# isl-org/Open3D-ML

Measured on AMD Instinct MI355X. Metric: point-cloud frames/sec (RandLA-Net SemanticKITTI inference: H2D + kNN pyramid + forward), higher is better.
Workload: dtype f32

## Files before the change

### include/ml3d_hip.h

```cpp
#ifndef ML3D_HIP_H
#define ML3D_HIP_H

#include <stddef.h>
#include <stdint.h>

#ifdef __cplusplus
extern "C" {
#endif

#define ML3D_OK 0
#define ML3D_E_INVALID (-1)
#define ML3D_E_WORKSPACE (-2)
#define ML3D_E_LAUNCH (-3)
#define ML3D_E_UNSUPPORTED (-4)

#define ML3D_ABI_VERSION 13
int ml3d_abi_version(void);

size_t ml3d_knn_workspace_bytes(int64_t n_points, int64_t n_queries, int64_t batch);

int ml3d_knn_search(const float* points, const int64_t* points_row_splits,
                    const float* queries, const int64_t* queries_row_splits,
                    int64_t batch, int64_t n_points, int64_t n_queries, int k,
                    int index_local, int32_t* out_index, float* out_dist2,
// ... 366 lines not shown
int ml3d_randla_knn_pyramid_ordered(const float* points, int64_t batch, int64_t n0, int num_layers,
                                    const int32_t* ratios_host, int k,
                                    int32_t* const* neighbor_idx_host, int32_t* const* interp_idx_host,
                                    int32_t* const* tile_order_host,
                                    void* workspace, size_t workspace_bytes, void* stream,
                                    const ml3d_trace* trace_host);

int ml3d_randla_forward_ordered(const ml3d_randla_desc* desc_host, const float* params,
                                const float* features, const float* points,
                                const int32_t* const* neighbor_idx_host,
                                const int32_t* const* interp_idx_host,
                                const int32_t* const* tile_order_host, float* out_scores,
                                void* workspace, size_t workspace_bytes, void* stream,
                                const ml3d_trace* trace_host);

int ml3d_gemm_tn(const float* a, int64_t lda, const float* b, int64_t ldb, int64_t m, int k, int n,
                 float* c, int64_t ldc, float* col_sums_a, void* stream);

size_t ml3d_batchnorm_train_workspace_bytes(int channels);

int ml3d_batchnorm_train_forward(const float* x, int64_t rows, int channels, const float* gamma,
                                 const float* beta, float eps, int act, float slope, float* y,
                                 float* save_mean, float* save_var, float* save_invstd,
                                 void* workspace, size_t workspace_bytes, void* stream);

int ml3d_batchnorm_train_backward(const float* x, const float* y, const float* grad_y, int64_t rows,
                                  int channels, const float* gamma, const float* save_mean,
                                  const float* save_invstd, int act, float slope, float* grad_x,
                                  float* grad_gamma, float* grad_beta, void* workspace,
                                  size_t workspace_bytes, void* stream);
// ... 118 lines not shown
```

### open3d-ml_amd/csrc/randla.hip

```cpp
#include <hip/hip_runtime.h>
#include <math.h>
#include <stdint.h>
#include <stdlib.h>

#include <type_traits>

#include "gemm.h"
#include <gfx950_ops.h>
#include "grid.h"
#include "ml3d_hip.h"

namespace ml3d {

static int64_t fuse_rows() {
#ifdef ML3D_TEST_HOOKS
    static const int64_t rows = [] { const char* e = getenv("ML3D_RANDLA_FUSE_ROWS"); return e ? (int64_t)atoll(e) : (int64_t)64 * 1024; }();
    return rows;
#else
    return 64 * 1024;
#endif
}

#ifndef ML3D_ATTN_B3
#define ML3D_ATTN_B3 3
// ... 24 lines not shown
struct LinArgs {
    const float* a0; int c0;
    const float* a1; int c1;
    const int32_t* gather;
    int64_t rows_per_item;
    int64_t a1_rows_per_item;
    const float* wt;
    const float* bias;
    const float* bias2;
    float* out;
    int64_t m_total;
    int cout;
    int act;
    float slope;
    void* pack_ws; size_t pack_bytes;
};

__global__ void __launch_bounds__(256)
head_fc0_mlp1(const float* __restrict__ x, int c0, const float* __restrict__ w0, const float* __restrict__ b0,
              const float* __restrict__ w1, const float* __restrict__ b1, int64_t m, float* __restrict__ feat,
              float* __restrict__ f1) {
    const int64_t i = (int64_t)blockIdx.x * blockDim.x + threadIdx.x;
    if (i >= m) return;
    float f[8], g[8];
#pragma unroll
    for (int c = 0; c < 8; ++c) f[c] = b0[c];
    const float* xr = x + i * c0;
    for (int j = 0; j < c0; ++j) {
        const float v = xr[j];
#pragma unroll
// ... 2226 lines not shown
    if (a.m_total <= 0) return 0;
    int64_t items = ((a.m_total + LIN_RM - 1) / LIN_RM) * a.cout;
    hipLaunchKernelGGL(linear_act, dim3((unsigned)((items + 255) / 256)), dim3(256), 0, st, a);
    return hipGetLastError() == hipSuccess ? 0 : ML3D_E_LAUNCH;
}

static int launch_linear_auto(const LinArgs& a, hipStream_t st) {
    if (!a.a1 && a.m_total >= fuse_rows()) {
        const ChainArgs c = chain_of(&a, 1);
        if (a.cout == 8 && mlp_shape_matches<ShapeLin16x8>(c)) return launch_mlp_wave_s<ShapeLin16x8, 8>(c, st);
        if (a.cout == 8 && mlp_shape_matches<ShapeLin8x8>(c)) return launch_mlp_wave_s<ShapeLin8x8, 8>(c, st);
        if (a.cout == 32 && mlp_shape_matches<ShapeLin64x32>(c)) return launch_mlp_wave_s<ShapeLin64x32, 8>(c, st);
        if (a.cout == 32 && mlp_shape_matches<ShapeLin32x32>(c)) return launch_mlp_wave_s<ShapeLin32x32, 8>(c, st);
        if (a.cout == 64 && mlp_shape_matches<ShapeLin32x64>(c)) return launch_mlp_wave_s<ShapeLin32x64, 8>(c, st);
    }
    if ((ML3D_LIN_B3_MINK) > 0 && a.pack_ws && !a.gather && a.c0 % 32 == 0 && (a.a1 ? a.c1 : 0) % 32 == 0 &&
        a.c0 + (a.a1 ? a.c1 : 0) >= (ML3D_LIN_B3_MINK) && a.cout % 4 == 0) {
        const int K = a.c0 + (a.a1 ? a.c1 : 0);
        const size_t need = gemm_pack_bf16x3_bytes(K, a.cout);
        if (need > 0 && need <= a.pack_bytes && gemm_pack_bf16x3(a.wt, K, a.cout, a.pack_ws, st) == 0) {
            const Epilogue ep = Epilogue::of(a.bias, a.act ? 1 : 0, a.slope).second_bias(a.bias2);
            const int rc = gemm_rows_bf16x3(a.a0, a.c0, a.c0, a.a1, a.c1, a.a1 ? a.c1 : 0, a.m_total, a.pack_ws, a.cout, ep, a.out,
                                            a.cout, nullptr, 0, st);
            if (rc != ML3D_E_UNSUPPORTED) return rc;
        }
    }
    if (a.c0 + a.c1 >= 8) {
        RowsA A;
        A.a = a.a0; A.lda = a.c0; A.k1 = a.c0;
        A.gather = a.a1 ? a.gather : nullptr; A.gather_stride = 1; A.a_rows = a.a1_rows_per_item;
        A.a2 = a.a1; A.lda2 = a.c1; A.k2 = a.a1 ? a.c1 : 0;
        A.gather_on_a2 = 1; A.g_rows_per_item = a.rows_per_item; A.g_src_rows_per_item = a.a1_rows_per_item;
        const Epilogue ep = Epilogue::of(a.bias, a.act ? 1 : 0, a.slope).second_bias(a.bias2);
        return gemm_rows(A, a.wt, a.m_total, a.cout, a.c0 + A.k2, ep, a.out, a.cout, nullptr, 0, st);
    }
    return launch_linear(a, st);
}
// ... 70 lines not shown
}

static size_t lin_pack_bytes(const ml3d_randla_desc* d) {
    size_t m = 0;
    int d_in = d->dim_features;
    for (int l = 0; l < d->num_layers; ++l) {
        const int dd = d->dim_output[l];
        const size_t a = gemm_pack_bf16x3_bytes(dd, dd), b = gemm_pack_bf16x3_bytes(dd + d_in, 2 * dd), c = gemm_pack_bf16x3_bytes(dd, dd / 2);
        m = a > m ? a : m; m = b > m ? b : m; m = c > m ? c : m;
        d_in = 2 * dd;
    }
    const size_t e = gemm_pack_bf16x3_bytes(d_in, d_in);
    return (e > m ? e : m) + 256;
}

static size_t fwd_ws_floats(const ml3d_randla_desc* d) {
    int64_t n[ML3D_RANDLA_MAX_LAYERS + 1];
    n[0] = d->num_points;
    for (int l = 0; l < d->num_layers; ++l) n[l + 1] = n[l] / d->sub_sampling_ratio[l];
    auto al = [](int64_t x) { return (x + 63) & ~(int64_t)63; };
    int64_t B = d->batch, f = 0;
    f += al(B * n[0] * d->dim_features);
    for (int l = 0; l < d->num_layers; ++l) {
        int64_t dd = d->dim_output[l], h = dd / 2;
        f += 2 * al(B * n[l] * h) + al(B * n[l] * 2 * dd) + al(B * n[l + 1] * 2 * dd) + 2 * al(B * n[l] * dd);
    }
    int64_t Dm = 2 * d->dim_output[d->num_layers - 1];
    f += al(B * n[d->num_layers] * Dm);
    int ed[ML3D_RANDLA_MAX_LAYERS + 1];
    enc_dims(d, ed);
    for (int i = 0; i < d->num_layers; ++i) {
        const int lev = d->num_layers - 1 - i, skip_c = ed[d->num_layers + 1 - i - 2];
        f += al(B * n[lev] * skip_c) + al(B * n[lev + 1] * skip_c);
    }
    f += al(B * n[0] * 64) + al(B * n[0] * 32);
    f += al((int64_t)(lin_pack_bytes(d) + 3) / 4) + 64;
    return (size_t)f;
}

}

using namespace ml3d;

extern "C" int ml3d_randla_param_layout(const ml3d_randla_desc* desc, int64_t* offsets_out, int max_slots) {
    if (!desc_ok(desc) || !offsets_out) return ML3D_E_INVALID;
    Layout L;
    make_layout(desc, &L);
    if (max_slots < L.n_slots + 1) return ML3D_E_INVALID;
    for (int i = 0; i <= L.n_slots; ++i) offsets_out[i] = L.off[i];
    return L.n_slots;
}

extern "C" size_t ml3d_randla_forward_workspace_bytes(const ml3d_randla_desc* desc) {
    if (!desc_ok(desc)) return 0;
    return fwd_ws_floats(desc) * 4 + 256;
}

extern "C" int ml3d_randla_forward(const ml3d_randla_desc* d, const float* params, const float* features,
                                   const float* points, const int32_t* const* neighbor_idx,
                                   const int32_t* const* interp_idx, float* out_scores, void* workspace,
                                   size_t workspace_bytes, void* stream) {
    return ml3d_randla_forward_traced(d, params, features, points, neighbor_idx, interp_idx, out_scores, workspace,
                                      workspace_bytes, stream, nullptr);
}

extern "C" int ml3d_randla_forward_traced(const ml3d_randla_desc* d, const float* params, const float* features,
                                          const float* points, const int32_t* const* neighbor_idx,
                                          const int32_t* const* interp_idx, float* out_scores, void* workspace,
                                          size_t workspace_bytes, void* stream, const ml3d_trace* trace) {
    return ml3d_randla_forward_ordered(d, params, features, points, neighbor_idx, interp_idx, nullptr, out_scores,
                                       workspace, workspace_bytes, stream, trace);
}

extern "C" int ml3d_randla_forward_ordered(const ml3d_randla_desc* d, const float* params, const float* features,
                                           const float* points, const int32_t* const* neighbor_idx,
                                           const int32_t* const* interp_idx, const int32_t* const* tile_order,
                                           float* out_scores, void* workspace, size_t workspace_bytes, void* stream,
                                           const ml3d_trace* trace) {
    if (!desc_ok(d) || !params || !features || !points || !neighbor_idx || !interp_idx || !out_scores)
        return ML3D_E_INVALID;
    if (d->num_neighbors != RK) return ML3D_E_UNSUPPORTED;
    if (workspace_bytes < ml3d_randla_forward_workspace_bytes(d)) return ML3D_E_WORKSPACE;
    hipStream_t st = (hipStream_t)stream;
    const Tracer T = {trace, st};
    const int Lr = d->num_layers;
    const int64_t B = d->batch;
    int64_t n[ML3D_RANDLA_MAX_LAYERS + 1];
    n[0] = d->num_points;
    for (int l = 0; l < Lr; ++l) n[l + 1] = n[l] / d->sub_sampling_ratio[l];
    if (n[Lr] < 1) return ML3D_E_INVALID;
    if (n[Lr - 1] < RK) return ML3D_E_UNSUPPORTED;
    Layout L;
    make_layout(d, &L);
    auto P = [&](int slot) { return params + L.off[slot]; };
    float* wsf = (float*)ws_align(workspace);
    auto take = [&](int64_t count) { float* p = wsf; wsf += (count + 63) & ~(int64_t)63; return p; };

    const size_t pack_bytes = lin_pack_bytes(d);
    void* pack_ws = take((int64_t)(pack_bytes + 3) / 4);
    auto lin = [&](const float* in, int k, int w, int b, float* out, int64_t rows, int cout, float slope,
                   const float* in1 = nullptr, int k1 = 0, int b2 = -1) {
        LinArgs a = {};
        a.pack_ws = pack_ws; a.pack_bytes = pack_bytes;
        a.a0 = in; a.c0 = k; a.a1 = in1; a.c1 = k1;
        a.wt = P(w); a.bias = b >= 0 ? P(b) : nullptr; a.bias2 = b2 >= 0 ? P(b2) : nullptr;
        a.out = out; a.m_total = rows; a.cout = cout; a.act = slope != 0.f; a.slope = slope;
        return a;
    };
    auto run = [&](int tag, const LinArgs& a) { return T.traced(tag, [&] { return launch_linear_auto(a, st); }); };
    int rc = 0;
    float* feat = take(B * n[0] * d->dim_features);
    float* f1_head = nullptr;
    if (d->dim_features == 8 && d->dim_output[0] == 16) {
        f1_head = take(B * n[0] * 8);
        const int64_t m = B * n[0];
        rc = T.traced(1000, [&] {
            hipLaunchKernelGGL(head_fc0_mlp1, dim3((unsigned)((m + 255) / 256)), dim3(256), 0, st, features, d->in_channels, P(0), P(1),
                               P(2), P(3), m, feat, f1_head);
// ... 100 lines not shown
    int cprev = Dm;
    for (int i = 0; i < Lr; ++i) {
        const int lev = Lr - 1 - i;
        const int skip_c = ed[Lr + 1 - i - 2];
        float* outp = take(B * n[lev] * skip_c);
        LinArgs a = lin(enc_keep[Lr + 1 - i - 2], skip_c, slot, slot + 1, outp, B * n[lev], skip_c, 0.2f, cur, cprev);
        a.gather = interp_idx[lev]; a.rows_per_item = n[lev]; a.a1_rows_per_item = n[lev + 1];
        if (i == Lr - 1) {
            LinArgs g[4] = {a};
            fc1(g + 1, outp, skip_c, nullptr, nullptr);
            const ChainArgs ch = chain_of(g, 4);
            if (mlp_shape_matches<ShapeDecFc1>(ch)) return T.traced(1200, [&] { return launch_chain_auto(ch, st); });
        }
        if (n[lev] >= 64 && (skip_c & 3) == 0 && (cprev & 3) == 0 && skip_c >= 8) {
            float* up = take(B * n[lev + 1] * skip_c);
            rc = T.traced(1100 + i, [&] {
                RowsA Au = {};
                Au.a = cur; Au.lda = cprev; Au.k1 = cprev;
                const int r = gemm_rows(Au, a.wt + (int64_t)skip_c * skip_c, B * n[lev + 1], skip_c, cprev, Epilogue{}, up, skip_c, nullptr, 0, st);
                if (r) return r;
                RowsA As = {};
                As.a = a.a0; As.lda = skip_c; As.k1 = skip_c;
                const Epilogue e1 = Epilogue::of(a.bias, 1, 0.2f).residual_rows(up, skip_c).gathered_residual(a.gather, 0, n[lev + 1], n[lev], n[lev + 1]);
                return gemm_rows(As, a.wt, a.m_total, skip_c, skip_c, e1, outp, skip_c, nullptr, 0, st);
            });
        } else {
            rc = run(1100 + i, a);
        }
        if (rc) return rc;
        slot += 2;
        cur = outp;
        cprev = skip_c;
    }
    float* t0 = take(B * n[0] * 64);
    float* t1 = take(B * n[0] * 32);
    LinArgs g[3];
    fc1(g, cur, cprev, t0, t1);
    return launch_linears(g, 3, true, T, 1200, st);
// ... 53 lines not shown
```

### open3d-ml_amd/ml3d/_abi.py

```python
import ctypes as C
import os

_HERE = os.path.dirname(os.path.abspath(__file__))
LIB_PATH = os.path.join(_HERE, "lib", "libml3d_hip.so")
MAX_LAYERS = 8
_lib = None

ERRORS = {-1: "invalid argument", -2: "workspace too small", -3: "HIP launch failed", -4: "unsupported configuration"}

ABI_VERSION = 13

SYMBOLS = [
    "ml3d_abi_version",
    "ml3d_knn_workspace_bytes",
    "ml3d_knn_search",
    "ml3d_radius_workspace_bytes",
    "ml3d_radius_count",
    "ml3d_radius_fill",
    "ml3d_radius_dense_workspace_bytes",
    "ml3d_radius_dense_gather",
    "ml3d_radius_dense_expand",
    "ml3d_ragged_to_dense",
    "ml3d_voxelize_workspace_bytes",
    "ml3d_voxelize_count",
# ... 44 lines not shown
    "ml3d_vote_update",
    "ml3d_randla_gather_max",
    "ml3d_randla_gather_max_backward",
    "ml3d_randla_attentive_pool",
    "ml3d_randla_attentive_pool_backward",
    "ml3d_argmax_labels",
    "ml3d_randla_pyramid_workspace_bytes",
    "ml3d_randla_knn_pyramid",
    "ml3d_randla_param_layout",
    "ml3d_randla_forward_workspace_bytes",
    "ml3d_randla_forward",
    "ml3d_randla_forward_traced",
    "ml3d_randla_knn_pyramid_traced",
    "ml3d_randla_knn_pyramid_ordered",
    "ml3d_randla_forward_ordered",
    "ml3d_gemm_tn",
    "ml3d_batchnorm_train_workspace_bytes", "ml3d_batchnorm_train_forward", "ml3d_batchnorm_train_backward",
    "ml3d_gather_rows", "ml3d_scatter_add_rows", "ml3d_gather_pool_backward",
    "ml3d_kpconv_deformed_weighted", "ml3d_kpconv_deformed_weighted_backward",
    "ml3d_kpconv_offset_regulariser_blocks", "ml3d_kpconv_offset_regulariser",
    "ml3d_randla_attention_stage", "ml3d_randla_attention_stage_backward_workspace_bytes", "ml3d_randla_attention_stage_backward",
    "ml3d_fps_workspace_bytes", "ml3d_furthest_point_sampling", "ml3d_pt_attention", "ml3d_pt_transition_down",
    "ml3d_pt_interpolate",
    "ml3d_pvcnn_voxel_coords", "ml3d_avg_voxelize_workspace_bytes", "ml3d_avg_voxelize", "ml3d_conv3d_ndhwc_bf16x3",
    "ml3d_trilinear_devoxelize", "ml3d_segment_max_rows_workspace_bytes", "ml3d_segment_max_rows",
    "ml3d_scn_build_workspace_bytes", "ml3d_scn_build", "ml3d_sparse_conv_bf16x3", "ml3d_scn_bn_relu",
    "ml3d_ball_query", "ml3d_pn2_sa_fused_supported", "ml3d_pn2_sa_mlp_max", "ml3d_pn2_group_rows", "ml3d_pn2_interpolate",
]


# ... 249 lines not shown
    lib.ml3d_randla_param_layout.restype = C.c_int
    lib.ml3d_randla_param_layout.argtypes = [C.POINTER(RandlaDesc), vp, i32]
    lib.ml3d_randla_forward_workspace_bytes.restype = sz
    lib.ml3d_randla_forward_workspace_bytes.argtypes = [C.POINTER(RandlaDesc)]
    lib.ml3d_randla_forward.restype = C.c_int
    lib.ml3d_randla_forward.argtypes = [C.POINTER(RandlaDesc), vp, vp, vp, vp, vp, vp, vp, sz, vp]
    lib.ml3d_randla_forward_traced.restype = C.c_int
    lib.ml3d_randla_forward_traced.argtypes = [C.POINTER(RandlaDesc), vp, vp, vp, vp, vp, vp, vp, sz, vp, C.POINTER(Trace)]
    lib.ml3d_randla_knn_pyramid_traced.restype = C.c_int
    lib.ml3d_randla_knn_pyramid_traced.argtypes = [vp, i64, i64, i32, vp, i32, vp, vp, vp, sz, vp, C.POINTER(Trace)]
    lib.ml3d_randla_knn_pyramid_ordered.restype = C.c_int
    lib.ml3d_randla_knn_pyramid_ordered.argtypes = [vp, i64, i64, i32, vp, i32, vp, vp, vp, vp, sz, vp, C.POINTER(Trace)]
    lib.ml3d_randla_forward_ordered.restype = C.c_int
    lib.ml3d_randla_forward_ordered.argtypes = [C.POINTER(RandlaDesc), vp, vp, vp, vp, vp, vp, vp, vp, sz, vp,
                                                C.POINTER(Trace)]
    return lib


def get():
    global _lib
    if _lib is None:
        if not os.path.exists(LIB_PATH):
            raise RuntimeError(
                "ml3d: %s is missing — build it with `python -c 'import __graft_entry__ as g; g.build()'` "
                "(hipcc --offload-arch=gfx950).  There is no CPU fallback." % LIB_PATH)
        lib = bind(C.CDLL(LIB_PATH))
        got = int(lib.ml3d_abi_version())
        if got != ABI_VERSION:
            raise RuntimeError("ml3d: %s has ABI version %d, this binding was written against %d (include/ml3d_hip.h) — rebuild "
                               "it with `python -c 'import __graft_entry__ as g; g.build()'`" % (LIB_PATH, got, ABI_VERSION))
# ... 69 lines not shown
```

### open3d-ml_amd/ml3d/engine.py

```python
import ctypes as C
import os

import torch

from . import _abi
from .ops import pyramid_sizes
from .torch.models import _randla_pack


class RandLAInferenceEngine:

    def __init__(self, cfg, state_dict, batch, num_points, device, tile_order=None):
        self.lib = _abi.get()
        if tile_order is None:
            env = (os.environ.get("ML3D_TILE_ORDER", "2") or "0").strip().lower()
            tile_order = True if env == "all" else int(env)
        self.tile_levels = (int(cfg["num_layers"]) if tile_order is True else int(tile_order or 0))
        self.tile_order = self.tile_levels > 0
        self.cfg = cfg
        self.device = torch.device(device)
        if self.device.type != "cuda":
            raise RuntimeError("RandLAInferenceEngine needs an MI355X device; there is no CPU fallback")
        self.B, self.N = int(batch), int(num_points)
        self.L = int(cfg["num_layers"])
        self.K = int(cfg["num_neighbors"])
        self.desc = _abi.make_desc(cfg, self.B, self.N)
        off = _abi.randla_param_offsets(self.lib, self.desc)
        self.params = torch.from_numpy(_randla_pack.pack(state_dict, cfg, off)).to(self.device)
        self.n = pyramid_sizes(self.N, cfg["sub_sampling_ratio"])
        dev = self.device
        self.nbr = [torch.empty((self.B, self.n[l], self.K), dtype=torch.int32, device=dev) for l in range(self.L)]
        self.itp = [torch.empty((self.B, self.n[l], 1), dtype=torch.int32, device=dev) for l in range(self.L)]
        self.scores = torch.empty((self.B, self.N, int(cfg["num_classes"])), dtype=torch.float32, device=dev)
        self.ratios = (C.c_int32 * self.L)(*[int(r) for r in cfg["sub_sampling_ratio"]])
        self.pyr_ws_bytes = self.lib.ml3d_randla_pyramid_workspace_bytes(self.B, self.N, self.L, self.ratios)
        self.fwd_ws_bytes = self.lib.ml3d_randla_forward_workspace_bytes(C.byref(self.desc))
        if self.pyr_ws_bytes == 0 or self.fwd_ws_bytes == 0:
            raise RuntimeError("RandLAInferenceEngine: invalid model/pyramid description")
        self.pyr_ws = torch.empty(self.pyr_ws_bytes, dtype=torch.uint8, device=dev)
        self.fwd_ws = torch.empty(self.fwd_ws_bytes, dtype=torch.uint8, device=dev)
        self._t_n = _abi.ptr_table([t.data_ptr() for t in self.nbr])
        self._t_i = _abi.ptr_table([t.data_ptr() for t in self.itp])
        self.order = [torch.empty(self.B * self.n[l], dtype=torch.int32, device=dev) if l < self.tile_levels else None
                      for l in range(self.L)] if self.tile_order else None
        self._t_o = _abi.ptr_table([0 if t is None else t.data_ptr() for t in self.order]) if self.tile_order else None

    def _check(self, points, features):
        if tuple(points.shape) != (self.B, self.N, 3) or points.dtype != torch.float32 or \
                not points.is_cuda or not points.is_contiguous():
            raise RuntimeError("engine: points must be a contiguous float32 CUDA tensor [%d, %d, 3]" % (self.B, self.N))
        if tuple(features.shape) != (self.B, self.N, int(self.cfg["in_channels"])) or \
                features.dtype != torch.float32 or not features.is_cuda or not features.is_contiguous():
            raise RuntimeError("engine: features must be a contiguous float32 CUDA tensor [B, N, in_channels]")

    def neighbors(self, points, trace=None):
        st = C.c_void_p(torch.cuda.current_stream().cuda_stream)
        rc = self.lib.ml3d_randla_knn_pyramid_ordered(points.data_ptr(), self.B, self.N, self.L, self.ratios, self.K,
                                                      self._t_n, self._t_i, self._t_o, self.pyr_ws.data_ptr(),
                                                      self.pyr_ws_bytes, st, trace)
        _abi.check(rc, "ml3d_randla_knn_pyramid")
        return self.nbr, self.itp

    def forward(self, points, features, trace=None):
        st = C.c_void_p(torch.cuda.current_stream().cuda_stream)
        rc = self.lib.ml3d_randla_forward_ordered(C.byref(self.desc), self.params.data_ptr(), features.data_ptr(),
                                                  points.data_ptr(), self._t_n, self._t_i, self._t_o,
                                                  self.scores.data_ptr(), self.fwd_ws.data_ptr(), self.fwd_ws_bytes, st,
                                                  trace)
        _abi.check(rc, "ml3d_randla_forward")
        return self.scores

    def step(self, points, features, knn_trace=None, fwd_trace=None):
        self._check(points, features)
        with torch.cuda.device(self.device):
            self.neighbors(points, knn_trace)
            return self.forward(points, features, fwd_trace)


class PipelinedRandLAEngine:

    def __init__(self, cfg, state_dict, batch, num_points, device):
        self.eng = [RandLAInferenceEngine(cfg, state_dict, batch, num_points, device) for _ in range(2)]
        self.eng[1].params = self.eng[0].params
        self.device = self.eng[0].device
        with torch.cuda.device(self.device):
            self.search = torch.cuda.Stream()
            self.compute = torch.cuda.Stream()
            self.knn_done = [torch.cuda.Event(), torch.cuda.Event()]
            self.fwd_done = [torch.cuda.Event(), torch.cuda.Event()]
            self.gate_tag = int(os.environ.get("ML3D_SEARCH_GATE", "9"))
            self.gate = [torch.cuda.Event(), torch.cuda.Event()]
            for g in self.gate:
                g.record()
        self.gate_rec = [None, None]
        self.i = 0
        self.n = self.eng[0].n

    def submit(self, points, features, knn_trace=None, fwd_trace=None, ready=None):
# ... 373 lines not shown
```

### open3d-ml_amd/ml3d/ops/__init__.py

```python
from ._gates import KnnResult, RadiusResult, VoxelizeResult
from .search import (knn_search, pyramid_sizes, randla_knn_pyramid, resolve_plans, fixed_radius_search,
                     radius_plan_dense, radius_fill_dense, radius_neighbors_dense, ragged_to_dense, _RadiusPlan,
                     _DenseRadiusPlan, kpconv_batch_build)
from .randla import randla_forward, GatherMaxFunction, AttentivePoolFunction
from .voxel import (voxelize, subsample_batch, subsample, rotate_points, grid_subsampling_plan,
                    batch_grid_subsampling, _SubsamplePlan)
from .kpconv import (kpconv_rigid, kpconv_deformable, linear, gather_pool, kpconv_weighted, kpconv_weighted_backward,
                     KPConvFunction)
from .detection import (pillar_features, conv2d_nhwc, pack_bf16x3, linear_bf16x3, deconv2d_nhwc, nhwc_to_nchw, nms, pointpillars_boxes,
                        iou_bev, iou_3d, topk_rows)
from .sampler import (nearest_to_center, argmax_labels, vote_update, device_patch, possibility_argmin,
                      device_patch_batch, sphere_select, device_sphere_batch)
from .train import (gemm_tn, LinearFunction, BatchNormActFunction, batch_norm_act, GatherRowsFunction, GatherPoolFunction,
                    AttentionStageFunction, attention_stage_supported, KPConvDeformedFunction, OffsetRegulariserFunction)
from .pointtransformer import furthest_point_sampling, pt_attention, pt_transition_down, pt_interpolate
from .pvcnn import (pvcnn_voxel_coords, avg_voxelize, pack_conv3d_weights, conv3d_ndhwc, trilinear_devoxelize,
                    segment_max_rows, linear_rows_bf16x3)
from .sparseconv import ScnPyramid, scn_build, pack_sparse_weights, sparse_conv, scn_bn_relu
from .pointnet2 import (ball_query, three_nn, three_interpolate, pn2_interpolate, pn2_sa_mlp_max, pack_sa_weights,
                        sa_fused)
```

### open3d-ml_amd/ml3d/ops/randla.py

```python
import ctypes as C

import numpy as np
import torch

from .. import _abi
from . import _gates
from ._gates import KnnResult, RadiusResult, VoxelizeResult, _splits, _splits_of_lengths


def _stream():
    return _gates._stream()


def _need_gpu(*tensors):
    return _gates._need_gpu(*tensors)


def _ws(nbytes, device):
    return _gates._ws(nbytes, device)

from .search import pyramid_sizes


def randla_forward(desc, params, features, points, neighbor_idx, interp_idx, out=None, workspace=None, tile_order=None):
    lib = _abi.get()
    _need_gpu(params, features, points, *neighbor_idx, *interp_idx)
    dev = points.device
    B, n0 = int(desc.batch), int(desc.num_points)
    if tuple(points.shape) != (B, n0, 3) or tuple(features.shape) != (B, n0, desc.in_channels):
        raise RuntimeError("randla_forward: points/features shape does not match the descriptor")
    for t in (points, features):
        if t.dtype != torch.float32 or not t.is_contiguous():
            raise RuntimeError("randla_forward: points/features must be contiguous float32")
    for t in list(neighbor_idx) + list(interp_idx):
        if t.dtype != torch.int32 or not t.is_contiguous():
            raise RuntimeError("randla_forward: index tensors must be contiguous int32")
    L, K = int(desc.num_layers), int(desc.num_neighbors)
    sizes = pyramid_sizes(n0, [int(desc.sub_sampling_ratio[i]) for i in range(L)])
    if len(neighbor_idx) != L or len(interp_idx) != L:
        raise RuntimeError("randla_forward: need %d neighbour and %d interpolation index tensors (got %d / %d)"
                           % (L, L, len(neighbor_idx), len(interp_idx)))
    for l in range(L):
        if tuple(neighbor_idx[l].shape) != (B, sizes[l], K):
            raise RuntimeError("randla_forward: neighbor_idx[%d] must be [%d, %d, %d], got %s"
                               % (l, B, sizes[l], K, tuple(neighbor_idx[l].shape)))
        if tuple(interp_idx[l].shape) not in ((B, sizes[l], 1), (B, sizes[l])):
            raise RuntimeError("randla_forward: interp_idx[%d] must be [%d, %d, 1], got %s"
                               % (l, B, sizes[l], tuple(interp_idx[l].shape)))
        if tile_order is not None and (l >= len(tile_order) or
                                       (tile_order[l] is not None and tile_order[l].numel() != B * sizes[l])):
            raise RuntimeError("randla_forward: tile_order[%d] must hold %d rows (or be None)" % (l, B * sizes[l]))
    if out is None:
        out = torch.empty((B, n0, desc.num_classes), dtype=torch.float32, device=dev)
    wsb = lib.ml3d_randla_forward_workspace_bytes(C.byref(desc))
    ws = workspace if workspace is not None else _ws(wsb, dev)
    if ws.numel() < wsb:
        raise RuntimeError("randla_forward: workspace too small")
    t_n = _abi.ptr_table([t.data_ptr() for t in neighbor_idx])
    t_i = _abi.ptr_table([t.data_ptr() for t in interp_idx])
    with torch.cuda.device(dev):
        if tile_order is not None:
            for t in tile_order:
                if t is not None and (t.dtype != torch.int32 or not t.is_contiguous() or t.device != dev):
                    raise RuntimeError("randla_forward: tile_order tensors must be contiguous int32 on the same device")
            t_o = _abi.ptr_table([0 if t is None else t.data_ptr() for t in tile_order])
            rc = lib.ml3d_randla_forward_ordered(C.byref(desc), params.data_ptr(), features.data_ptr(), points.data_ptr(),
                                                 t_n, t_i, t_o, out.data_ptr(), ws.data_ptr(), ws.numel(), _stream(), None)
        else:
            rc = lib.ml3d_randla_forward(C.byref(desc), params.data_ptr(), features.data_ptr(), points.data_ptr(),
                                         t_n, t_i, out.data_ptr(), ws.data_ptr(), ws.numel(), _stream())
    _abi.check(rc, "ml3d_randla_forward")
    return out


class GatherMaxFunction(torch.autograd.Function):

    @staticmethod
    def forward(ctx, features, neighbor_idx, n_out):
        lib = _abi.get()
        _need_gpu(features, neighbor_idx)
# ... 59 lines not shown
```

### open3d-ml_amd/ml3d/torch/models/randlanet.py

```python
import os

import numpy as np
import torch
import torch.nn as nn

from ... import _abi
from ... import ops
from . import _randla_pack
from ._datapath import GpuSearchTree, preprocess_segmentation
from ._multicloud import CloudSlots, PinnedUpload, check_many_args


class SharedMLP(nn.Module):

    def __init__(self, in_channels, out_channels, transpose=False, bn=True, activation_fn=None):
        super().__init__()
        conv = nn.ConvTranspose2d if transpose else nn.Conv2d
        self.conv = conv(in_channels, out_channels, kernel_size=1)
        self.batch_norm = nn.BatchNorm2d(out_channels, eps=1e-6, momentum=0.01) if bn else None
        self.activation_fn = activation_fn


class LocalSpatialEncoding(nn.Module):
    def __init__(self, dim_in, dim_out):
# ... 66 lines not shown
                                 SharedMLP(32, cfg.num_classes, bn=False))
        self._packed = None
        self._engines = {}
        self.use_graphs = os.environ.get("ML3D_RANDLA_GRAPHS", "0") == "1"
        self.eval()

    def _apply(self, fn, *a, **k):
        self._packed = None
        return super()._apply(fn, *a, **k)

    def load_state_dict(self, *a, **k):
        self._packed = None
        return super().load_state_dict(*a, **k)

    def packed_params(self, device):
        if self._packed is None or self._packed[0] != device:
            desc = _abi.make_desc(self.cfg, 1, max(self.cfg.num_points, 1))
            off = _abi.randla_param_offsets(_abi.get(), desc)
            buf = _randla_pack.pack(self.state_dict(), self.cfg, off)
            self._packed = (device, torch.from_numpy(buf).to(device))
        return self._packed[1]

    def invalidate_packed(self):
        self._packed = None

    def neighbor_pyramid(self, points):
        return ops.randla_knn_pyramid(points, self.cfg.sub_sampling_ratio, self.cfg.num_neighbors)

    def forward(self, inputs):
        if self.training:
            return self._forward_train(inputs)
        dev = self.device
        _abi.require_gpu(dev, "RandLANet.forward")
        fast = self._forward_graphed(inputs)
        if fast is not None:
# ... 3 lines not shown
        feat = inputs['features'].to(dev, torch.float32).contiguous()
        if 'neighbor_indices' in inputs and 'interp_idx' in inputs:
            nbr = [t.to(dev).to(torch.int32).contiguous() for t in inputs['neighbor_indices']]
            itp = [t.to(dev).to(torch.int32).contiguous() for t in inputs['interp_idx']]
            if 'sub_idx' in inputs:
                for l, (sub, nb) in enumerate(zip(inputs['sub_idx'], nbr)):
                    if getattr(sub, '_ml3d_prefix_of_neighbors', False) and sub.shape[-2] <= nb.shape[-2]:
                        continue
                    sub = sub.to(dev)
                    if sub.shape[-2] > nb.shape[-2] or not torch.equal(sub.to(torch.int32), nb[..., :sub.shape[-2], :]):
                        raise RuntimeError("RandLANet.forward: sub_idx[%d] is not the prefix of neighbor_indices[%d]" % (l, l))
        else:
            nbr, itp = self.neighbor_pyramid(pts)
        B, N, _ = pts.shape
        desc = _abi.make_desc(self.cfg, B, N)
        return ops.randla_forward(desc, self.packed_params(dev), feat, pts, nbr, itp)

    def _forward_graphed(self, inputs):
        st = getattr(self, '_dev_loop', None)
        feats = inputs.get('features') if isinstance(inputs, dict) else None
        mark = getattr(feats, '_ml3d_arena', None)
        if st is None or mark is None or not getattr(self, 'use_graphs', True) or st.get('fwd_failed') or st.get('layout') is None:
            return None
        arena, lay_id = mark
        lay, nbytes = st['layout']
        if lay_id != id(lay) or arena.numel() != nbytes or feats.dim() != 3 or feats.shape[0] != 1:
            return None
        base, L = arena.data_ptr(), int(self.cfg.num_layers)
        coords = inputs['coords'][0] if isinstance(inputs['coords'], (list, tuple)) else inputs['coords']
        try:
            ok = feats.data_ptr() == base + lay['feats'][0] and coords.data_ptr() == base + lay['pts'][0] and \
                all(inputs['neighbor_indices'][l].data_ptr() == base + lay['nbr%d' % l][0] and
                    inputs['interp_idx'][l].data_ptr() == base + lay['itp%d' % l][0] for l in range(L))
        except Exception:
            ok = False
        if not ok:
            return None
        dev = self.device
        fg = st.get('fwd_graph')
        params = self.packed_params(dev)
        if fg is not None and fg['params'] is not params:
            fg = None
        if fg is None:
            try:
                with torch.cuda.device(dev):
                    a_in = torch.empty(nbytes, dtype=torch.uint8, device=dev)
                    a_in.copy_(arena)
                    v = self._arena_views(a_in, lay)
                    k = int(self.cfg.num_points)
                    desc = _abi.make_desc(self.cfg, 1, k)
                    nbr = [v['nbr%d' % l] for l in range(L)]
                    itp = [v['itp%d' % l] for l in range(L)]
                    scores = torch.empty((1, k, int(self.cfg.num_classes)), dtype=torch.float32, device=dev)
                    run = lambda: ops.randla_forward(desc, params, v['feats'][None], v['pts'][None], nbr, itp, out=scores)
                    side = torch.cuda.Stream()
# ... 491 lines not shown
```

Baseline: 7560.

## Pre-pack RandLA-Net weights into bf16x3 planes once at load time

```diff
diff --git a/include/ml3d_hip.h b/include/ml3d_hip.h
--- a/include/ml3d_hip.h
+++ b/include/ml3d_hip.h
@@ -404,6 +404,19 @@
                                 void* workspace, size_t workspace_bytes, void* stream,
                                 const ml3d_trace* trace_host);
 
+size_t ml3d_randla_prepared_bytes(const ml3d_randla_desc* desc_host);
+int ml3d_randla_prepare(const ml3d_randla_desc* desc_host, const float* params, void* prepared, size_t prepared_bytes,
+                        void* stream);
+size_t ml3d_randla_prepared_forward_bytes(const ml3d_randla_desc* desc_host);
+int ml3d_randla_forward_prepared(const ml3d_randla_desc* desc_host, const float* params,
+                                 const float* features, const float* points,
+                                 const int32_t* const* neighbor_idx_host,
+                                 const int32_t* const* interp_idx_host,
+                                 const int32_t* const* tile_order_host, float* out_scores,
+                                 void* workspace, size_t workspace_bytes, void* stream,
+                                 const ml3d_trace* trace_host, const void* prepared, size_t prepared_bytes,
+                                 int32_t lin_min_k, int32_t dec_min_k);
+
 int ml3d_gemm_tn(const float* a, int64_t lda, const float* b, int64_t ldb, int64_t m, int k, int n,
                  float* c, int64_t ldc, float* col_sums_a, void* stream);
 
diff --git a/open3d-ml_amd/csrc/randla.hip b/open3d-ml_amd/csrc/randla.hip
--- a/open3d-ml_amd/csrc/randla.hip
+++ b/open3d-ml_amd/csrc/randla.hip
@@ -62,6 +62,7 @@
     int act;
     float slope;
     void* pack_ws; size_t pack_bytes;
+    const void* planes; int b3_min_k;
 };
 
 __global__ void __launch_bounds__(256)
@@ -2318,13 +2319,18 @@
         if (a.cout == 32 && mlp_shape_matches<ShapeLin32x32>(c)) return launch_mlp_wave_s<ShapeLin32x32, 8>(c, st);
         if (a.cout == 64 && mlp_shape_matches<ShapeLin32x64>(c)) return launch_mlp_wave_s<ShapeLin32x64, 8>(c, st);
     }
-    if ((ML3D_LIN_B3_MINK) > 0 && a.pack_ws && !a.gather && a.c0 % 32 == 0 && (a.a1 ? a.c1 : 0) % 32 == 0 &&
-        a.c0 + (a.a1 ? a.c1 : 0) >= (ML3D_LIN_B3_MINK) && a.cout % 4 == 0) {
+    if (!a.gather && a.c0 % 32 == 0 && (a.a1 ? a.c1 : 0) % 32 == 0 && a.cout % 4 == 0) {
         const int K = a.c0 + (a.a1 ? a.c1 : 0);
-        const size_t need = gemm_pack_bf16x3_bytes(K, a.cout);
-        if (need > 0 && need <= a.pack_bytes && gemm_pack_bf16x3(a.wt, K, a.cout, a.pack_ws, st) == 0) {
+        const void* planes = nullptr;
+        if (a.planes) {
+            if (K >= a.b3_min_k) planes = a.planes;
+        } else if ((ML3D_LIN_B3_MINK) > 0 && a.pack_ws && K >= (ML3D_LIN_B3_MINK)) {
+            const size_t need = gemm_pack_bf16x3_bytes(K, a.cout);
+            if (need > 0 && need <= a.pack_bytes && gemm_pack_bf16x3(a.wt, K, a.cout, a.pack_ws, st) == 0) planes = a.pack_ws;
+        }
+        if (planes) {
             const Epilogue ep = Epilogue::of(a.bias, a.act ? 1 : 0, a.slope).second_bias(a.bias2);
-            const int rc = gemm_rows_bf16x3(a.a0, a.c0, a.c0, a.a1, a.c1, a.a1 ? a.c1 : 0, a.m_total, a.pack_ws, a.cout, ep, a.out,
+            const int rc = gemm_rows_bf16x3(a.a0, a.c0, a.c0, a.a1, a.c1, a.a1 ? a.c1 : 0, a.m_total, planes, a.cout, ep, a.out,
                                             a.cout, nullptr, 0, st);
             if (rc != ML3D_E_UNSUPPORTED) return rc;
         }
@@ -2425,7 +2431,7 @@
     return (e > m ? e : m) + 256;
 }
 
-static size_t fwd_ws_floats(const ml3d_randla_desc* d) {
+static size_t fwd_ws_floats(const ml3d_randla_desc* d, bool pack) {
     int64_t n[ML3D_RANDLA_MAX_LAYERS + 1];
     n[0] = d->num_points;
     for (int l = 0; l < d->num_layers; ++l) n[l + 1] = n[l] / d->sub_sampling_ratio[l];
@@ -2445,13 +2451,87 @@
         f += al(B * n[lev] * skip_c) + al(B * n[lev + 1] * skip_c);
     }
     f += al(B * n[0] * 64) + al(B * n[0] * 32);
-    f += al((int64_t)(lin_pack_bytes(d) + 3) / 4) + 64;
-    return (size_t)f;
+    if (pack) f += al((int64_t)(lin_pack_bytes(d) + 3) / 4);
+    return (size_t)f + 64;
+}
+
+constexpr int PREP_LIN_MINK = 256;
+constexpr int PREP_DEC_MINK = INT32_MAX;
+constexpr int PREP_MINK = 64;
+
+struct PrepEntry { int slot, row0, K, N; void* planes; };
+struct RandlaPrepared {
+    int n;
+    PrepEntry e[6 * ML3D_RANDLA_MAX_LAYERS + 1 + 2 * ML3D_RANDLA_MAX_LAYERS];
+    const void* find(int slot, int row0, int K, int N) const {
+        for (int i = 0; i < n; ++i)
+            if (e[i].slot == slot && e[i].row0 == row0 && e[i].K == K && e[i].N == N) return e[i].planes;
+        return nullptr;
+    }
+};
+
+static RandlaPrepared randla_prepared_layout(WsLayout& L, const ml3d_randla_desc* d) {
+    RandlaPrepared P;
+    P.n = 0;
+    auto add = [&](int slot, int row0, int K, int N) {
+        if (K < PREP_MINK || (N & 3) != 0 || gemm_pack_bf16x3_bytes(K, N) == 0) return;
+        P.e[P.n++] = {slot, row0, K, N, L.take<char>(gemm_pack_bf16x3_bytes(K, N))};
+    };
+    int d_in = d->dim_features;
+    for (int l = 0; l < d->num_layers; ++l) {
+        const int dd = d->dim_output[l], h = dd / 2, sb = 2 + 18 * l;
+        add(sb + 0, 0, d_in, h);
+        add(sb + 4, 0, h, dd);
+        add(sb + 6, 0, dd, h);
+        add(sb + 10, 0, h, dd);
+        add(sb + 12, 0, dd, dd);
+        add(sb + 14, 0, dd + d_in, 2 * dd);
+        d_in = 2 * dd;
+    }
+    int slot = 2 + 18 * d->num_layers;
+    add(slot, 0, d_in, d_in);
+    slot += 2;
+    int ed[ML3D_RANDLA_MAX_LAYERS + 1];
+    enc_dims(d, ed);
+    int cprev = d_in;
+    for (int i = 0; i < d->num_layers; ++i) {
+        const int skip_c = ed[d->num_layers + 1 - i - 2];
+        add(slot, 0, skip_c, skip_c);
+        add(slot, skip_c, cprev, skip_c);
+        slot += 2;
+        cprev = skip_c;
+    }
+    return P;
 }
 
 }
 
 using namespace ml3d;
+
+extern "C" size_t ml3d_randla_prepared_bytes(const ml3d_randla_desc* desc) {
+    if (!desc_ok(desc)) return 0;
+    return ws_bytes_of(randla_prepared_layout, desc);
+}
+
+extern "C" int ml3d_randla_prepare(const ml3d_randla_desc* d, const float* params, void* prepared, size_t prepared_bytes,
+                                   void* stream) {
+    if (!desc_ok(d) || !params || !prepared) return ML3D_E_INVALID;
+    RandlaPrepared P;
+    if (!ws_carve(prepared, prepared_bytes, &P, randla_prepared_layout, d)) return ML3D_E_WORKSPACE;
+    Layout L;
+    make_layout(d, &L);
+    for (int i = 0; i < P.n; ++i) {
+        const PrepEntry& e = P.e[i];
+        const int rc = gemm_pack_bf16x3(params + L.off[e.slot] + (int64_t)e.row0 * e.N, e.K, e.N, e.planes, (hipStream_t)stream);
+        if (rc) return rc;
+    }
+    return 0;
+}
+
+extern "C" size_t ml3d_randla_prepared_forward_bytes(const ml3d_randla_desc* desc) {
+    if (!desc_ok(desc)) return 0;
+    return fwd_ws_floats(desc, false) * 4 + 256;
+}
 
 extern "C" int ml3d_randla_param_layout(const ml3d_randla_desc* desc, int64_t* offsets_out, int max_slots) {
     if (!desc_ok(desc) || !offsets_out) return ML3D_E_INVALID;
@@ -2464,7 +2544,7 @@
 
 extern "C" size_t ml3d_randla_forward_workspace_bytes(const ml3d_randla_desc* desc) {
     if (!desc_ok(desc)) return 0;
-    return fwd_ws_floats(desc) * 4 + 256;
+    return fwd_ws_floats(desc, true) * 4 + 256;
 }
 
 extern "C" int ml3d_randla_forward(const ml3d_randla_desc* d, const float* params, const float* features,
@@ -2483,15 +2563,41 @@
                                        workspace, workspace_bytes, stream, trace);
 }
 
+static int randla_forward(const ml3d_randla_desc* d, const float* params, const float* features, const float* points,
+                          const int32_t* const* neighbor_idx, const int32_t* const* interp_idx, const int32_t* const* tile_order,
+                          float* out_scores, void* workspace, size_t workspace_bytes, void* stream, const ml3d_trace* trace,
+                          const RandlaPrepared* prep, int lin_min_k, int dec_min_k);
+
 extern "C" int ml3d_randla_forward_ordered(const ml3d_randla_desc* d, const float* params, const float* features,
                                            const float* points, const int32_t* const* neighbor_idx,
                                            const int32_t* const* interp_idx, const int32_t* const* tile_order,
                                            float* out_scores, void* workspace, size_t workspace_bytes, void* stream,
                                            const ml3d_trace* trace) {
+    return randla_forward(d, params, features, points, neighbor_idx, interp_idx, tile_order, out_scores, workspace, workspace_bytes,
+                          stream, trace, nullptr, 0, 0);
+}
+
+extern "C" int ml3d_randla_forward_prepared(const ml3d_randla_desc* d, const float* params, const float* features,
+                                            const float* points, const int32_t* const* neighbor_idx,
+                                            const int32_t* const* interp_idx, const int32_t* const* tile_order,
+                                            float* out_scores, void* workspace, size_t workspace_bytes, void* stream,
+                                            const ml3d_trace* trace, const void* prepared, size_t prepared_bytes,
+                                            int32_t lin_min_k, int32_t dec_min_k) {
+    if (!desc_ok(d) || !prepared || lin_min_k < 0 || dec_min_k < 0) return ML3D_E_INVALID;
+    RandlaPrepared P;
+    if (!ws_carve((void*)prepared, prepared_bytes, &P, randla_prepared_layout, d)) return ML3D_E_WORKSPACE;
+    return randla_forward(d, params, features, points, neighbor_idx, interp_idx, tile_order, out_scores, workspace, workspace_bytes,
+                          stream, trace, &P, lin_min_k ? lin_min_k : PREP_LIN_MINK, dec_min_k ? dec_min_k : PREP_DEC_MINK);
+}
+
+static int randla_forward(const ml3d_randla_desc* d, const float* params, const float* features, const float* points,
+                          const int32_t* const* neighbor_idx, const int32_t* const* interp_idx, const int32_t* const* tile_order,
+                          float* out_scores, void* workspace, size_t workspace_bytes, void* stream, const ml3d_trace* trace,
+                          const RandlaPrepared* prep, int lin_min_k, int dec_min_k) {
     if (!desc_ok(d) || !params || !features || !points || !neighbor_idx || !interp_idx || !out_scores)
         return ML3D_E_INVALID;
     if (d->num_neighbors != RK) return ML3D_E_UNSUPPORTED;
-    if (workspace_bytes < ml3d_randla_forward_workspace_bytes(d)) return ML3D_E_WORKSPACE;
+    if (workspace_bytes < fwd_ws_floats(d, !prep) * 4 + 256) return ML3D_E_WORKSPACE;
     hipStream_t st = (hipStream_t)stream;
     const Tracer T = {trace, st};
     const int Lr = d->num_layers;
@@ -2507,12 +2613,13 @@
     float* wsf = (float*)ws_align(workspace);
     auto take = [&](int64_t count) { float* p = wsf; wsf += (count + 63) & ~(int64_t)63; return p; };
 
-    const size_t pack_bytes = lin_pack_bytes(d);
-    void* pack_ws = take((int64_t)(pack_bytes + 3) / 4);
+    const size_t pack_bytes = prep ? 0 : lin_pack_bytes(d);
+    void* pack_ws = prep ? nullptr : take((int64_t)(pack_bytes + 3) / 4);
     auto lin = [&](const float* in, int k, int w, int b, float* out, int64_t rows, int cout, float slope,
                    const float* in1 = nullptr, int k1 = 0, int b2 = -1) {
         LinArgs a = {};
         a.pack_ws = pack_ws; a.pack_bytes = pack_bytes;
+        if (prep) { a.planes = prep->find(w, 0, k + k1, cout); a.b3_min_k = lin_min_k; }
         a.a0 = in; a.c0 = k; a.a1 = in1; a.c1 = k1;
         a.wt = P(w); a.bias = b >= 0 ? P(b) : nullptr; a.bias2 = b2 >= 0 ? P(b2) : nullptr;
         a.out = out; a.m_total = rows; a.cout = cout; a.act = slope != 0.f; a.slope = slope;
@@ -2643,14 +2750,25 @@
         }
         if (n[lev] >= 64 && (skip_c & 3) == 0 && (cprev & 3) == 0 && skip_c >= 8) {
             float* up = take(B * n[lev + 1] * skip_c);
+            const void* up_planes = prep && cprev >= dec_min_k ? prep->find(slot, skip_c, cprev, skip_c) : nullptr;
+            const void* skip_planes = prep && skip_c >= dec_min_k ? prep->find(slot, 0, skip_c, skip_c) : nullptr;
             rc = T.traced(1100 + i, [&] {
-                RowsA Au = {};
-                Au.a = cur; Au.lda = cprev; Au.k1 = cprev;
-                const int r = gemm_rows(Au, a.wt + (int64_t)skip_c * skip_c, B * n[lev + 1], skip_c, cprev, Epilogue{}, up, skip_c, nullptr, 0, st);
+                int r = up_planes ? gemm_rows_bf16x3(cur, cprev, cprev, nullptr, 0, 0, B * n[lev + 1], up_planes, skip_c, Epilogue{}, up,
+                                                     skip_c, nullptr, 0, st)
+                                  : ML3D_E_UNSUPPORTED;
+                if (r == ML3D_E_UNSUPPORTED) {
+                    RowsA Au = {};
+                    Au.a = cur; Au.lda = cprev; Au.k1 = cprev;
+                    r = gemm_rows(Au, a.wt + (int64_t)skip_c * skip_c, B * n[lev + 1], skip_c, cprev, Epilogue{}, up, skip_c, nullptr, 0, st);
+                }
                 if (r) return r;
+                const Epilogue e1 = Epilogue::of(a.bias, 1, 0.2f).residual_rows(up, skip_c).gathered_residual(a.gather, 0, n[lev + 1], n[lev], n[lev + 1]);
+                r = skip_planes ? gemm_rows_bf16x3(a.a0, skip_c, skip_c, nullptr, 0, 0, a.m_total, skip_planes, skip_c, e1, outp, skip_c,
+                                                   nullptr, 0, st)
+                                : ML3D_E_UNSUPPORTED;
+                if (r != ML3D_E_UNSUPPORTED) return r;
                 RowsA As = {};
                 As.a = a.a0; As.lda = skip_c; As.k1 = skip_c;
-                const Epilogue e1 = Epilogue::of(a.bias, 1, 0.2f).residual_rows(up, skip_c).gathered_residual(a.gather, 0, n[lev + 1], n[lev], n[lev + 1]);
                 return gemm_rows(As, a.wt, a.m_total, skip_c, skip_c, e1, outp, skip_c, nullptr, 0, st);
             });
         } else {
diff --git a/open3d-ml_amd/ml3d/_abi.py b/open3d-ml_amd/ml3d/_abi.py
--- a/open3d-ml_amd/ml3d/_abi.py
+++ b/open3d-ml_amd/ml3d/_abi.py
@@ -82,6 +82,7 @@
     "ml3d_randla_knn_pyramid_traced",
     "ml3d_randla_knn_pyramid_ordered",
     "ml3d_randla_forward_ordered",
+    "ml3d_randla_prepared_bytes", "ml3d_randla_prepare", "ml3d_randla_prepared_forward_bytes", "ml3d_randla_forward_prepared",
     "ml3d_gemm_tn",
     "ml3d_batchnorm_train_workspace_bytes", "ml3d_batchnorm_train_forward", "ml3d_batchnorm_train_backward",
     "ml3d_gather_rows", "ml3d_scatter_add_rows", "ml3d_gather_pool_backward",
@@ -361,6 +362,15 @@
     lib.ml3d_randla_forward_ordered.restype = C.c_int
     lib.ml3d_randla_forward_ordered.argtypes = [C.POINTER(RandlaDesc), vp, vp, vp, vp, vp, vp, vp, vp, sz, vp,
                                                 C.POINTER(Trace)]
+    lib.ml3d_randla_prepared_bytes.restype = sz
+    lib.ml3d_randla_prepared_bytes.argtypes = [C.POINTER(RandlaDesc)]
+    lib.ml3d_randla_prepare.restype = C.c_int
+    lib.ml3d_randla_prepare.argtypes = [C.POINTER(RandlaDesc), vp, vp, sz, vp]
+    lib.ml3d_randla_prepared_forward_bytes.restype = sz
+    lib.ml3d_randla_prepared_forward_bytes.argtypes = [C.POINTER(RandlaDesc)]
+    lib.ml3d_randla_forward_prepared.restype = C.c_int
+    lib.ml3d_randla_forward_prepared.argtypes = [C.POINTER(RandlaDesc), vp, vp, vp, vp, vp, vp, vp, vp, sz, vp,
+                                                 C.POINTER(Trace), vp, sz, i32, i32]
     return lib
 
 
diff --git a/open3d-ml_amd/ml3d/engine.py b/open3d-ml_amd/ml3d/engine.py
--- a/open3d-ml_amd/ml3d/engine.py
+++ b/open3d-ml_amd/ml3d/engine.py
@@ -5,12 +5,13 @@
 
 from . import _abi
 from .ops import pyramid_sizes
+from .ops.randla import RandlaWeights, prepared_routing
 from .torch.models import _randla_pack
 
 
 class RandLAInferenceEngine:
 
-    def __init__(self, cfg, state_dict, batch, num_points, device, tile_order=None):
+    def __init__(self, cfg, state_dict, batch, num_points, device, tile_order=None, weights=None):
         self.lib = _abi.get()
         if tile_order is None:
             env = (os.environ.get("ML3D_TILE_ORDER", "2") or "0").strip().lower()
@@ -26,7 +27,11 @@
         self.K = int(cfg["num_neighbors"])
         self.desc = _abi.make_desc(cfg, self.B, self.N)
         off = _abi.randla_param_offsets(self.lib, self.desc)
-        self.params = torch.from_numpy(_randla_pack.pack(state_dict, cfg, off)).to(self.device)
+        if weights is None:
+            with torch.cuda.device(self.device):
+                weights = RandlaWeights(self.desc, torch.from_numpy(_randla_pack.pack(state_dict, cfg, off)).to(self.device))
+        self.weights = weights
+        self.routing = prepared_routing()
         self.n = pyramid_sizes(self.N, cfg["sub_sampling_ratio"])
         dev = self.device
         self.nbr = [torch.empty((self.B, self.n[l], self.K), dtype=torch.int32, device=dev) for l in range(self.L)]
@@ -34,7 +39,8 @@
         self.scores = torch.empty((self.B, self.N, int(cfg["num_classes"])), dtype=torch.float32, device=dev)
         self.ratios = (C.c_int32 * self.L)(*[int(r) for r in cfg["sub_sampling_ratio"]])
         self.pyr_ws_bytes = self.lib.ml3d_randla_pyramid_workspace_bytes(self.B, self.N, self.L, self.ratios)
-        self.fwd_ws_bytes = self.lib.ml3d_randla_forward_workspace_bytes(C.byref(self.desc))
+        self.fwd_ws_bytes = (self.lib.ml3d_randla_prepared_forward_bytes if self.weights.prepared is not None else
+                             self.lib.ml3d_randla_forward_workspace_bytes)(C.byref(self.desc))
         if self.pyr_ws_bytes == 0 or self.fwd_ws_bytes == 0:
             raise RuntimeError("RandLAInferenceEngine: invalid model/pyramid description")
         self.pyr_ws = torch.empty(self.pyr_ws_bytes, dtype=torch.uint8, device=dev)
@@ -45,6 +51,10 @@
                       for l in range(self.L)] if self.tile_order else None
         self._t_o = _abi.ptr_table([0 if t is None else t.data_ptr() for t in self.order]) if self.tile_order else None
 
+    @property
+    def params(self):
+        return self.weights.params
+
     def _check(self, points, features):
         if tuple(points.shape) != (self.B, self.N, 3) or points.dtype != torch.float32 or \
                 not points.is_cuda or not points.is_contiguous():
@@ -63,10 +73,18 @@
 
     def forward(self, points, features, trace=None):
         st = C.c_void_p(torch.cuda.current_stream().cuda_stream)
-        rc = self.lib.ml3d_randla_forward_ordered(C.byref(self.desc), self.params.data_ptr(), features.data_ptr(),
-                                                  points.data_ptr(), self._t_n, self._t_i, self._t_o,
-                                                  self.scores.data_ptr(), self.fwd_ws.data_ptr(), self.fwd_ws_bytes, st,
-                                                  trace)
+        w = self.weights
+        if w.prepared is not None:
+            rc = self.lib.ml3d_randla_forward_prepared(C.byref(self.desc), w.params.data_ptr(), features.data_ptr(),
+                                                       points.data_ptr(), self._t_n, self._t_i, self._t_o,
+                                                       self.scores.data_ptr(), self.fwd_ws.data_ptr(), self.fwd_ws_bytes, st,
+                                                       trace, w.prepared.data_ptr(), w.prepared.numel(), self.routing[0],
+                                                       self.routing[1])
+        else:
+            rc = self.lib.ml3d_randla_forward_ordered(C.byref(self.desc), w.params.data_ptr(), features.data_ptr(),
+                                                      points.data_ptr(), self._t_n, self._t_i, self._t_o,
+                                                      self.scores.data_ptr(), self.fwd_ws.data_ptr(), self.fwd_ws_bytes, st,
+                                                      trace)
         _abi.check(rc, "ml3d_randla_forward")
         return self.scores
 
@@ -80,8 +98,8 @@
 class PipelinedRandLAEngine:
 
     def __init__(self, cfg, state_dict, batch, num_points, device):
-        self.eng = [RandLAInferenceEngine(cfg, state_dict, batch, num_points, device) for _ in range(2)]
-        self.eng[1].params = self.eng[0].params
+        self.eng = [RandLAInferenceEngine(cfg, state_dict, batch, num_points, device)]
+        self.eng.append(RandLAInferenceEngine(cfg, state_dict, batch, num_points, device, weights=self.eng[0].weights))
         self.device = self.eng[0].device
         with torch.cuda.device(self.device):
             self.search = torch.cuda.Stream()
diff --git a/open3d-ml_amd/ml3d/ops/__init__.py b/open3d-ml_amd/ml3d/ops/__init__.py
--- a/open3d-ml_amd/ml3d/ops/__init__.py
+++ b/open3d-ml_amd/ml3d/ops/__init__.py
@@ -2,7 +2,7 @@
 from .search import (knn_search, pyramid_sizes, randla_knn_pyramid, resolve_plans, fixed_radius_search,
                      radius_plan_dense, radius_fill_dense, radius_neighbors_dense, ragged_to_dense, _RadiusPlan,
                      _DenseRadiusPlan, kpconv_batch_build)
-from .randla import randla_forward, GatherMaxFunction, AttentivePoolFunction
+from .randla import randla_forward, randla_prepare, RandlaWeights, GatherMaxFunction, AttentivePoolFunction
 from .voxel import (voxelize, subsample_batch, subsample, rotate_points, grid_subsampling_plan,
                     batch_grid_subsampling, _SubsamplePlan)
 from .kpconv import (kpconv_rigid, kpconv_deformable, linear, gather_pool, kpconv_weighted, kpconv_weighted_backward,
diff --git a/open3d-ml_amd/ml3d/ops/randla.py b/open3d-ml_amd/ml3d/ops/randla.py
--- a/open3d-ml_amd/ml3d/ops/randla.py
+++ b/open3d-ml_amd/ml3d/ops/randla.py
@@ -1,4 +1,5 @@
 import ctypes as C
+import os
 
 import numpy as np
 import torch
@@ -22,8 +23,47 @@
 from .search import pyramid_sizes
 
 
-def randla_forward(desc, params, features, points, neighbor_idx, interp_idx, out=None, workspace=None, tile_order=None):
+def prepared_routing():
+    env = os.environ.get("ML3D_RANDLA_PREP_MINK", "").strip()
+    if not env:
+        return 0, 0
+    lin, dec = (int(v) for v in env.split(","))
+    return lin, dec
+
+
+def prepared_enabled():
+    return os.environ.get("ML3D_RANDLA_PREPARED", "1").strip() != "0"
+
+
+class RandlaWeights:
+
+    def __init__(self, desc, params, prepare=True):
+        _need_gpu(params)
+        if params.dtype != torch.float32 or not params.is_contiguous():
+            raise RuntimeError("RandlaWeights: params must be a contiguous float32 tensor")
+        self.params = params
+        self.prepared = randla_prepare(desc, params) if prepare and prepared_enabled() else None
+
+
+def randla_prepare(desc, params):
     lib = _abi.get()
+    _need_gpu(params)
+    nbytes = int(lib.ml3d_randla_prepared_bytes(C.byref(desc)))
+    if nbytes == 0:
+        raise RuntimeError("randla_prepare: invalid model description")
+    blob = _ws(nbytes, params.device)
+    with torch.cuda.device(params.device):
+        rc = lib.ml3d_randla_prepare(C.byref(desc), params.data_ptr(), blob.data_ptr(), blob.numel(), _stream())
+    _abi.check(rc, "ml3d_randla_prepare")
+    return blob
+
+
+def randla_forward(desc, params, features, points, neighbor_idx, interp_idx, out=None, workspace=None, tile_order=None,
+                   routing=None):
+    lib = _abi.get()
+    prepared = None
+    if isinstance(params, RandlaWeights):
+        params, prepared = params.params, params.prepared
     _need_gpu(params, features, points, *neighbor_idx, *interp_idx)
     dev = points.device
     B, n0 = int(desc.batch), int(desc.num_points)
@@ -52,18 +92,25 @@
             raise RuntimeError("randla_forward: tile_order[%d] must hold %d rows (or be None)" % (l, B * sizes[l]))
     if out is None:
         out = torch.empty((B, n0, desc.num_classes), dtype=torch.float32, device=dev)
-    wsb = lib.ml3d_randla_forward_workspace_bytes(C.byref(desc))
+    wsb = (lib.ml3d_randla_forward_workspace_bytes if prepared is None else lib.ml3d_randla_prepared_forward_bytes)(C.byref(desc))
     ws = workspace if workspace is not None else _ws(wsb, dev)
     if ws.numel() < wsb:
         raise RuntimeError("randla_forward: workspace too small")
     t_n = _abi.ptr_table([t.data_ptr() for t in neighbor_idx])
     t_i = _abi.ptr_table([t.data_ptr() for t in interp_idx])
     with torch.cuda.device(dev):
+        t_o = None
         if tile_order is not None:
             for t in tile_order:
                 if t is not None and (t.dtype != torch.int32 or not t.is_contiguous() or t.device != dev):
                     raise RuntimeError("randla_forward: tile_order tensors must be contiguous int32 on the same device")
             t_o = _abi.ptr_table([0 if t is None else t.data_ptr() for t in tile_order])
+        if prepared is not None:
+            lin_k, dec_k = prepared_routing() if routing is None else routing
+            rc = lib.ml3d_randla_forward_prepared(C.byref(desc), params.data_ptr(), features.data_ptr(), points.data_ptr(),
+                                                  t_n, t_i, t_o, out.data_ptr(), ws.data_ptr(), ws.numel(), _stream(), None,
+                                                  prepared.data_ptr(), prepared.numel(), int(lin_k), int(dec_k))
+        elif tile_order is not None:
             rc = lib.ml3d_randla_forward_ordered(C.byref(desc), params.data_ptr(), features.data_ptr(), points.data_ptr(),
                                                  t_n, t_i, t_o, out.data_ptr(), ws.data_ptr(), ws.numel(), _stream(), None)
         else:
diff --git a/open3d-ml_amd/ml3d/torch/models/randlanet.py b/open3d-ml_amd/ml3d/torch/models/randlanet.py
--- a/open3d-ml_amd/ml3d/torch/models/randlanet.py
+++ b/open3d-ml_amd/ml3d/torch/models/randlanet.py
@@ -104,11 +104,15 @@
         return super().load_state_dict(*a, **k)
 
     def packed_params(self, device):
+        return self.prepared_weights(device).params
+
+    def prepared_weights(self, device):
         if self._packed is None or self._packed[0] != device:
             desc = _abi.make_desc(self.cfg, 1, max(self.cfg.num_points, 1))
             off = _abi.randla_param_offsets(_abi.get(), desc)
             buf = _randla_pack.pack(self.state_dict(), self.cfg, off)
-            self._packed = (device, torch.from_numpy(buf).to(device))
+            with torch.cuda.device(device):
+                self._packed = (device, ops.RandlaWeights(desc, torch.from_numpy(buf).to(device)))
         return self._packed[1]
 
     def invalidate_packed(self):
@@ -142,7 +146,7 @@
             nbr, itp = self.neighbor_pyramid(pts)
         B, N, _ = pts.shape
         desc = _abi.make_desc(self.cfg, B, N)
-        return ops.randla_forward(desc, self.packed_params(dev), feat, pts, nbr, itp)
+        return ops.randla_forward(desc, self.prepared_weights(dev), feat, pts, nbr, itp)
 
     def _forward_graphed(self, inputs):
         st = getattr(self, '_dev_loop', None)
@@ -166,7 +170,7 @@
             return None
         dev = self.device
         fg = st.get('fwd_graph')
-        params = self.packed_params(dev)
+        params = self.prepared_weights(dev)
         if fg is not None and fg['params'] is not params:
             fg = None
         if fg is None:
```

After: 7555. About the same (-0.1%).
